# SreenivasVRao/SuperSloMo-VideoInterpolation-PyTorch

Hardware: AMD Instinct MI355X
Metric: interpolated 1280x720 frames/sec (higher is better)
Workload: dtype f32

## Files before the change

include/ssm_hip.h:

```cpp
#ifndef SSM_HIP_H
#define SSM_HIP_H

#include <stddef.h>

#ifdef __cplusplus
extern "C" {
#endif

#define SSM_PADX 4
#define SSM_PADY 3
#define SSM_TAIL_SLACK_FLOATS (1 << 16)

#define SSM_OK 0
#define SSM_E_ARG (-1)
#define SSM_E_LAUNCH (-2)
#define SSM_E_UNSUPPORTED (-3)

#define SSM_FLAG_LRELU 1
#define SSM_FLAG_FP16_FAST 2
#define SSM_FLAG_Q8 4
#define SSM_FLAG_MASK 8

typedef struct ssm_view {
    float *ptr;
// ... 49 lines not shown

int ssm_wino_splitk_plan(int Cin, int Cout, int B, int H, int W, int ups, int BN, int *KS);
int ssm_wino_conv2d_splitk_fwd(ssm_view x1, int C1, ssm_view x2, int C2, const float *w_packed, const float *bias_packed, ssm_view part,
                               int KS, int ups, int B, int H, int W, int Cout, int BN, void *stream);
int ssm_splitk_finish_fwd(ssm_view part, int KS, ssm_view y, ssm_view pool, ssm_view add, int add_div, int B, int C, int H, int W,
                          float slope, int flags, void *stream);
int ssm_conv_splitk_plan(int k, int Cin, int Cout, int B, int H, int W, int *KS);
int ssm_splitk_enable(int wino, int conv);
int ssm_conv2d_splitk_fwd(ssm_view x1, int C1, ssm_view x2, int C2, const float *w_packed, const float *bias_packed, ssm_view part,
                          int KS, int B, int H, int W, int Cout, int k, void *stream);
int ssm_wino_conv2d_add_fwd(ssm_view x1, int C1, ssm_view x2, int C2, const float *w_packed, const float *bias_packed, ssm_view y,
                            ssm_view pool, ssm_view add, int add_div, int B, int H, int W, int Cout, float slope, int flags,
                            void *stream);
int ssm_wino_conv2d_ups_add_fwd(ssm_view a, int C1, ssm_view b, int C2, const float *w_packed, const float *bias_packed, ssm_view y,
                                ssm_view add, int add_div, int B, int H, int W, int Cout, float slope, int flags, void *stream);

int ssm_wino4_plan(int Cin, int Cout, int B, int H, int W, int ups, int *kind, int *BN, int *CK);
int ssm_wino4_preferred(int Cin, int Cout, int B, int H, int W, int ups);
double ssm_wino_estimate(int Cin, int Cout, int B, int H, int W, int ups);
int ssm_wino4_force_kind(int kind);
size_t ssm_wino4_packed_weight_floats(int Cout, int Cin);
int ssm_wino4_pack_weights(const float *w_oihw, const float *bias, float *w_packed, float *bias_packed, int Cout, int Cin, void *stream);
int ssm_wino4_conv2d_add_fwd(ssm_view x1, int C1, ssm_view x2, int C2, const float *w_packed, const float *bias_packed, ssm_view y,
                             ssm_view pool, ssm_view add, int add_div, int B, int H, int W, int Cout, float slope, int flags,
                             void *stream);
int ssm_wino4_conv2d_ups_add_fwd(ssm_view a, int C1, ssm_view b, int C2, const float *w_packed, const float *bias_packed, ssm_view y,
                                 ssm_view add, int add_div, int B, int H, int W, int Cout, float slope, int flags, void *stream);
#define SSM_WINO4_BORDER_TH 16
#define SSM_WINO4_BORDER_TW 32
int ssm_wino4_conv2d_shuffle_fwd(ssm_view x1, int C1, ssm_view x2, int C2, const float *w_packed, const float *bias_packed, ssm_view y, int B,
                                 int H, int W, int Cout4, float slope, int flags, void *stream);
int ssm_wino4_conv2d_ups_border_fwd(ssm_view a, int C1, ssm_view b, int C2, const float *w_packed, const float *bias_packed, ssm_view y, int B,
                                    int H, int W, int Cout, float slope, int flags, void *stream);

int ssm_wino1d_plan(int k, int Cin, int Cout, int B, int H, int W, int *kind, int *BN, int *CK);
int ssm_wino1d_force_kind(int kind);
size_t ssm_wino1d_packed_weight_floats(int Cout, int CinP, int k, int BN);
int ssm_wino1d_pack_weights(const float *w_oihw, const float *bias, float *w_packed, float *bias_packed, int Cout, int Cin,
                            int CinP, int k, int BN, void *stream);
int ssm_wino1d_conv2d_add_fwd(ssm_view x, int Cin, const float *w_packed, const float *bias_packed, ssm_view y, ssm_view pool,
                              ssm_view add, int add_div, int B, int H, int W, int Cout, int k, float slope, int flags, void *stream);

int ssm_wino7_plan(int Cin, int Cout, int B, int H, int W, int *kind);
int ssm_wino7_force_kind(int kind);
size_t ssm_wino7_packed_weight_floats(int Cout, int Cin);
int ssm_wino7_pack_weights(const float *w_oihw, const float *bias, float *w_packed, float *bias_packed, int Cout, int Cin, void *stream);
int ssm_wino7_conv2d_add_fwd(ssm_view x, int Cin, const float *w_packed, const float *bias_packed, ssm_view y, ssm_view pool,
                             ssm_view add, int add_div, int B, int H, int W, int Cout, float slope, int flags, void *stream);

int ssm_wino5_plan(int Cin, int Cout, int B, int H, int W, int *kind);
int ssm_wino5_force_kind(int kind);
size_t ssm_wino5_packed_weight_floats(int Cout, int CinP);
int ssm_wino5_pack_weights(const float *w_oihw, const float *bias, float *w_packed, float *bias_packed, int Cout, int Cin, int CinP,
                           void *stream);
int ssm_wino5_conv2d_add_fwd(ssm_view x, int Cin, const float *w_packed, const float *bias_packed, ssm_view y, ssm_view pool,
                             ssm_view add, int add_div, int B, int H, int W, int Cout, float slope, int flags, void *stream);

enum { SSM_PACK_DIRECT = 0, SSM_PACK_WINO = 1, SSM_PACK_WINO1D = 2, SSM_PACK_WINO4 = 3, SSM_PACK_WINO7 = 4, SSM_PACK_WINO5 = 5 };
typedef struct {
    const float *w;
    const float *bias;
    float *wp, *bp;
    int Cout, Cin, CinP, k, BN, algo, transposed, nbias;
    long long first, total;
} ssm_pack32_job;
int ssm_pack32_weights_batch(const ssm_pack32_job *jobs_device, int n_jobs, long long total_elements, void *stream);
// ... 199 lines not shown
```

superslomo-videointerpolation-pytorch_amd/ssm_amd/engine.py:

```python
import os

import torch

from . import hipbind as hb
from .weights import RECURRENT_HIDDEN, RECURRENT_LAYERS, param_key, recurrent_convs, unet_layers


class KernelTimer:

    def __init__(self):
        self.spans = []

    def span(self, family, name, flops=0.0, nbytes=0.0, issued=None):
        e0, e1 = torch.cuda.Event(enable_timing=True), torch.cuda.Event(enable_timing=True)
        self.spans.append((family, name, flops, nbytes, e0, e1, flops if issued is None else issued))
        return e0, e1

    def summary(self):
        out = {}
        for fam, name, fl, nb, e0, e1, isd in self.spans:
            d = out.setdefault(fam, {"ms": 0.0, "flops": 0.0, "issued": 0.0, "bytes": 0.0, "launches": 0, "by_name": {}})
            ms = e0.elapsed_time(e1)
            d["ms"] += ms
            d["flops"] += fl
# ... 5 lines not shown
            n[1] += fl
            n[2] += 1
        return out


MODES = ("f32", "f32w", "f16x3", "f16", "f16f8")


def base_mode(mode):
    return "f32" if mode == "f32w" else mode


HOIST_PAIR_PARTS = os.environ.get("SSM_HOIST", "1") != "0"

WINO_SKIP = frozenset(n for n in os.environ.get("SSM_WINO_SKIP", "").split(",") if n)

WINO1D = os.environ.get("SSM_WINO1D", "57")


WINO7 = os.environ.get("SSM_WINO7", "1")
WINO5 = os.environ.get("SSM_WINO5", "1")


WINO4 = os.environ.get("SSM_WINO4", "1")


TRAIN_WINO4 = os.environ.get("SSM_TRAIN_WINO4", "1")
TRAIN_FWD_BLOCKED = os.environ.get("SSM_TRAIN_FWD_BLOCKED", "1")


WINO4_SUBPIXEL = tuple(n for n in os.environ.get("SSM_WINO4_SUBPIXEL", "conv11a").split(",") if n not in ("", "0"))


def wino4_enabled(name):
    return WINO4 not in ("0", "") and (WINO4 == "1" or name in WINO4.split(","))


def wino1d_enabled(k):
    return k in (5, 7) and str(k) in WINO1D


def choose_algo(name, ci, co, k, nb, h, w, ups, wino, wino1d, wino4=None, blocked2d=None):
    skip = name in WINO_SKIP or "all" in WINO_SKIP or name == "final_conv"
    wino4 = wino1d if wino4 is None else wino4
    blocked2d = wino1d if blocked2d is None else blocked2d
    if blocked2d and not skip and k == 7 and WINO7 not in ("0", "") and hb.wino7_supported(ci, co, h, w, k):
        return "wino7"
    if blocked2d and not skip and k == 5 and WINO5 not in ("0", "") and ci % 4 == 0 and hb.wino5_supported(ci, co, h, w, k):
        return "wino5"
    if wino1d and not skip and wino1d_enabled(k) and hb.wino1d_supported(ci, co, h, w, k):
        return "wino1d"
    if wino and not skip and hb.wino_supported(ci, co, h, w, k):
        if (wino4 and wino4_enabled(name) and hb.wino4_supported(ci, co, h, w, k)
                and (WINO4 != "1" or hb.wino4_preferred(ci, co, nb, h, w, ups))):
            return "wino4"
        return "wino"
    return "direct"


_ALGO_CLASS = {"direct": lambda: hb.PackedConv, "wino": lambda: hb.PackedWino, "wino4": lambda: hb.PackedWino4, "wino1d": lambda: hb.PackedWino1d,
               "wino7": lambda: hb.PackedWino7, "wino5": lambda: hb.PackedWino5}
ISSUED_FACTOR = {"direct": lambda k: 1.0, "wino": lambda k: 16.0 / 36.0, "wino4": lambda k: 36.0 / 144.0,
                 "wino1d": lambda k: 8.0 / 14.0 if k == 7 else 8.0 / 20.0, "wino7": lambda k: 196.0 / 784.0,
                 "wino5": lambda k: 64.0 / 400.0}


def issued_factor(pk):
    return ISSUED_FACTOR.get(getattr(pk, "algo", "direct"), ISSUED_FACTOR["direct"])(pk.k)


def conv_fn(pk, ups=False):
    if pk.algo == "wino7":
        return hb.conv2d_wino7
    if pk.algo == "wino5":
        return hb.conv2d_wino5
    if pk.algo == "wino1d":
        return hb.conv2d_wino1d
    if pk.algo == "wino4":
        return hb.conv2d_ups_wino4 if ups else hb.conv2d_wino4
    if pk.algo == "wino":
        return hb.conv2d_ups_wino if ups else hb.conv2d_wino
    return hb.conv2d_ups if ups else hb.conv2d


POOLED = ("conv1b", "conv2b", "conv3b", "conv4b", "conv5b")
_SCALE = (("conv10", 2), ("conv11", 1), ("conv1", 1), ("conv2", 2), ("conv3", 4), ("conv4", 8), ("conv5", 16),
          ("conv6", 32), ("conv7", 16), ("conv8", 8), ("conv9", 4), ("fuse_conv", 1), ("final_conv", 1))


def layer_scale(name):
    for prefix, s in _SCALE:
        if name.startswith(prefix):
            return s
    raise KeyError(name)


class UNetPlan:
    timer = None
    RESCALE_EVERY = int(os.environ.get("SSM_RESCALE_EVERY", "256"))
    fast_layers = frozenset()

    DECODER = ("conv7a", "conv7b", "conv8a", "conv8b", "conv9a", "conv9b", "conv10a", "conv10b", "conv11a", "conv11b",
               "fuse_conv", "final_conv")
    ENCODER_T = ("c1", "c2", "c3", "c4", "c5", "c6")
# ... 90 lines not shown
        batchable = self.q8 and all(t.is_cuda and t.dtype == torch.float32 and t.is_contiguous() for t in tensors)
        self._refreshes = getattr(self, "_refreshes", 0) + 1
        if self._refreshes % self.RESCALE_EVERY == 0:
            self.scales, self._pack = {}, None
        if batchable and getattr(self, "_pack", None) is not None and self._pack[0] == hb.PackBatch.key(tensors):
            self._pack[1].run()
            if getattr(self, "rnn", None) is not None:
                self.rnn.refresh_weights(state_dict)
            return
        batch32 = (not self.hl8 and not self.hoist and os.environ.get("SSM_PACK_BATCH", "1") != "0"
                   and all(t.is_cuda and t.dtype == torch.float32 and t.is_contiguous() for t in tensors))
        if batch32 and getattr(self, "_pack32", None) is not None and self._pack32[0] == hb.PackBatch.key(tensors):
            self._pack32[1].run()
            if "final_conv" in self.layers:
                self.final_wb = (state_dict[param_key("final_conv", "weight")].detach(), state_dict[param_key("final_conv", "bias")].detach())
            if getattr(self, "rnn", None) is not None:
                self.rnn.refresh_weights(state_dict)
            return
        for name, (ci, co, k) in self.layers.items():
            w = state_dict[param_key(name, "weight")].to(device=self.device, dtype=torch.float32)
            b = state_dict[param_key(name, "bias")].to(device=self.device, dtype=torch.float32)
            if check_shapes:
                assert tuple(w.shape) == (co, ci, k, k), "%s: weight shape %s != %s" % (name, tuple(w.shape), (co, ci, k, k))
            s = layer_scale(name)
            if name == "final_conv":
                self.final_wb = (w.contiguous(), b.contiguous())
            if self.hl8:
                self.pk[name] = hb.PackedConv16(w, b, self.W // s, q8=self.q8, ups=self.fuse_up and name in self.UPS,
                                                scale=self.scales.get(name))
                self.scales.setdefault(name, self.pk[name].scale)
            else:
                nb = self.Bd if name in self.DECODER else self.B
                ups = self.fuse_up and name in self.UPS
                cls = _ALGO_CLASS[choose_algo(name, ci, co, k, nb, self.H // s, self.W // s, ups, self.wino, self.wino1d, self.wino4, self.blocked2d)]()
                if self.hoist and name == "conv1a":
                    zb = torch.zeros_like(b)
                    self.pk[name] = cls(w[:, 3:13].contiguous(), b, nb, self.H // s, self.W // s)
                    self.pk_pair[name] = cls(torch.cat([w[:, 13:16], w[:, 0:3]], 1).contiguous(), zb, self.hoist[0], self.H // s, self.W // s)
                elif self.hoist and name == "conv7a" and self.cross:
                    zb = torch.zeros_like(b)
                    self.pk[name] = cls(w[:, :512].contiguous(), b, nb, self.H // s, self.W // s, ups=ups)
                    self.pk_pair[name] = cls(w[:, 512:].contiguous(), zb, self.hoist[0], self.H // s, self.W // s, ups=ups)
                elif (ups and cls is hb.PackedWino4 and name in WINO4_SUBPIXEL and not self.twins
                      and hb.subpixel_wino4_supported(ci, co, self.H // s, self.W // s)):
                    self.pk[name] = hb.PackedSubpixelWino4(w, b, nb, self.H // s, self.W // s)
                    batch32 = False
                else:
                    self.pk[name] = cls(w, b, nb, self.H // s, self.W // s, pool=name in POOLED, ups=ups)
        for pkk in list(self.pk.values()) + list(getattr(self, "pk_pair", {}).values()):
            if self.wino and isinstance(pkk, hb.PackedConv):
                pkk.split_ok = True
        self._pack32 = None
        if batch32:
            entries = [(self.pk[name], state_dict[param_key(name, "weight")], state_dict[param_key(name, "bias")], False)
                       for name in self.layers]
            self._pack32 = (hb.PackBatch.key(tensors), hb.PackBatch32(entries, self.device))
        self._pack = None
        if batchable:
            entries = [(self.pk[name], state_dict[param_key(name, "weight")], state_dict[param_key(name, "bias")], False)
                       for name in self.layers]
            self._pack = (hb.PackBatch.key(tensors), hb.PackBatch(entries, self.device))
        if getattr(self, "rnn", None) is not None:
            self.rnn.refresh_weights(state_dict)

    def _v(self, name, **kw):
        if self._b0 and name in self.ENCODER_T:
            kw["b0"] = self._b0
        return self.t[name].view(**kw)

    def _conv(self, name, src, dst, pool=None, src2=None, lrelu=True):
        pk = self.pk[name]
        s = self.t[src]
        d = self.t[dst]
        c2 = self.t[src2].C if src2 else 0
        tm = self.timer
        if tm is not None:
            fl = 2.0 * self._Bcur * s.H * s.W * pk.cout * pk.cin * pk.k * pk.k
            e0, e1 = tm.span("conv", "s%d.%s" % (self.stage, name), fl, issued=fl * issued_factor(pk))
            e0.record()
        v = self._v
        if self.hl8:
            final = name == "final_conv"
            y32 = v(dst) if final else (self.f32[dst].view() if self.twins else None)
            hb.conv2d_hl8(v(src), s.G * 8, v(src2) if src2 else None, c2, pk, None if final else v(dst),
# ... 593 lines not shown
```

superslomo-videointerpolation-pytorch_amd/ssm_amd/hipbind.py:

```python
import ctypes
import os
import threading

import torch

_HERE = os.path.dirname(os.path.abspath(__file__))
LIB_PATH = os.environ.get("SSM_HIP_LIB") or os.path.join(os.path.dirname(_HERE), "lib", "libssm_hip.so")

SSM_PADX = 4
SSM_PADY = 3
SSM_TAIL_SLACK_FLOATS = 1 << 16
SSM_FLAG_LRELU = 1
SSM_FLAG_MASK = 8


class SsmView(ctypes.Structure):
    _fields_ = [("ptr", ctypes.c_void_p), ("sb", ctypes.c_longlong), ("sc", ctypes.c_longlong),
                ("sh", ctypes.c_int)]


NULL_VIEW = SsmView(None, 0, 0, 0)


class SsmHView(ctypes.Structure):
# ... 19 lines not shown
    "ssm_pack_weights": (_c_int, [_vp, _vp, _vp, _vp, _c_int, _c_int, _c_int, _c_int, _c_int, _vp]),
    "ssm_conv2d_fwd": (_c_int, [SsmView, _c_int, SsmView, _c_int, _vp, _vp, SsmView, SsmView, _c_int, _c_int,
                                _c_int, _c_int, _c_int, _c_float, _c_int, _vp]),
    "ssm_conv2d_add_fwd": (_c_int, [SsmView, _c_int, SsmView, _c_int, _vp, _vp, SsmView, SsmView, SsmView, _c_int, _c_int, _c_int,
                                    _c_int, _c_int, _c_int, _c_float, _c_int, _vp]),
    "ssm_conv2d_ups_add_fwd": (_c_int, [SsmView, _c_int, SsmView, _c_int, _vp, _vp, SsmView, SsmView, _c_int, _c_int, _c_int, _c_int,
                                        _c_int, _c_float, _c_int, _vp]),
    "ssm_wino_conv2d_add_fwd": (_c_int, [SsmView, _c_int, SsmView, _c_int, _vp, _vp, SsmView, SsmView, SsmView, _c_int, _c_int, _c_int,
                                         _c_int, _c_int, _c_float, _c_int, _vp]),
    "ssm_wino_conv2d_ups_add_fwd": (_c_int, [SsmView, _c_int, SsmView, _c_int, _vp, _vp, SsmView, SsmView, _c_int, _c_int, _c_int, _c_int,
                                             _c_int, _c_float, _c_int, _vp]),
    "ssm_wino_plan": (_c_int, [_c_int, _c_int, _c_int, _c_int, _c_int, _c_int, _ip, _ip, _ip]),
    "ssm_wino_splitk_plan": (_c_int, [_c_int, _c_int, _c_int, _c_int, _c_int, _c_int, _c_int, _ip]),
    "ssm_conv_splitk_plan": (_c_int, [_c_int, _c_int, _c_int, _c_int, _c_int, _c_int, _ip]),
    "ssm_conv2d_splitk_fwd": (_c_int, [SsmView, _c_int, SsmView, _c_int, _vp, _vp, SsmView, _c_int, _c_int, _c_int, _c_int, _c_int, _c_int, _vp]),
    "ssm_wino_conv2d_splitk_fwd": (_c_int, [SsmView, _c_int, SsmView, _c_int, _vp, _vp, SsmView, _c_int, _c_int, _c_int, _c_int, _c_int, _c_int,
                                            _c_int, _vp]),
    "ssm_splitk_finish_fwd": (_c_int, [SsmView, _c_int, SsmView, SsmView, SsmView, _c_int, _c_int, _c_int, _c_int, _c_int, _c_float, _c_int, _vp]),
    "ssm_wino_force_kind": (_c_int, [_c_int]),
    "ssm_wino_packed_weight_floats": (_sz, [_c_int, _c_int, _c_int]),
    "ssm_wino_pack_weights": (_c_int, [_vp, _vp, _vp, _vp, _c_int, _c_int, _c_int, _vp]),
    "ssm_pack32_weights_batch": (_c_int, [_vp, _c_int, ctypes.c_longlong, _vp]),
    "ssm_pack32_wino_tiles_batch": (_c_int, [_vp, _c_int, ctypes.c_longlong, _c_int, _vp]),
    "ssm_wino4_plan": (_c_int, [_c_int, _c_int, _c_int, _c_int, _c_int, _c_int, _ip, _ip, _ip]),
    "ssm_wino4_force_kind": (_c_int, [_c_int]),
    "ssm_wino4_preferred": (_c_int, [_c_int, _c_int, _c_int, _c_int, _c_int, _c_int]),
    "ssm_wino_estimate": (ctypes.c_double, [_c_int, _c_int, _c_int, _c_int, _c_int, _c_int]),
    "ssm_wino4_packed_weight_floats": (_sz, [_c_int, _c_int]),
    "ssm_wino4_pack_weights": (_c_int, [_vp, _vp, _vp, _vp, _c_int, _c_int, _vp]),
    "ssm_wino4_conv2d_add_fwd": (_c_int, [SsmView, _c_int, SsmView, _c_int, _vp, _vp, SsmView, SsmView, SsmView, _c_int, _c_int, _c_int,
                                          _c_int, _c_int, _c_float, _c_int, _vp]),
    "ssm_wino4_conv2d_ups_add_fwd": (_c_int, [SsmView, _c_int, SsmView, _c_int, _vp, _vp, SsmView, SsmView, _c_int, _c_int, _c_int, _c_int,
                                              _c_int, _c_float, _c_int, _vp]),
    "ssm_wino4_conv2d_shuffle_fwd": (_c_int, [SsmView, _c_int, SsmView, _c_int, _vp, _vp, SsmView, _c_int, _c_int, _c_int, _c_int, _c_float, _c_int, _vp]),
    "ssm_wino4_conv2d_ups_border_fwd": (_c_int, [SsmView, _c_int, SsmView, _c_int, _vp, _vp, SsmView, _c_int, _c_int, _c_int, _c_int, _c_float, _c_int,
                                                 _vp]),
    "ssm_wino1d_plan": (_c_int, [_c_int, _c_int, _c_int, _c_int, _c_int, _c_int, _ip, _ip, _ip]),
    "ssm_wino1d_force_kind": (_c_int, [_c_int]),
    "ssm_wino1d_packed_weight_floats": (_sz, [_c_int, _c_int, _c_int, _c_int]),
    "ssm_wino1d_pack_weights": (_c_int, [_vp, _vp, _vp, _vp, _c_int, _c_int, _c_int, _c_int, _c_int, _vp]),
    "ssm_wino1d_conv2d_add_fwd": (_c_int, [SsmView, _c_int, _vp, _vp, SsmView, SsmView, SsmView, _c_int, _c_int, _c_int, _c_int, _c_int,
                                           _c_int, _c_float, _c_int, _vp]),
    "ssm_wino5_plan": (_c_int, [_c_int, _c_int, _c_int, _c_int, _c_int, _ip]),
    "ssm_wino5_force_kind": (_c_int, [_c_int]),
    "ssm_wino5_packed_weight_floats": (_sz, [_c_int, _c_int]),
    "ssm_wino5_pack_weights": (_c_int, [_vp, _vp, _vp, _vp, _c_int, _c_int, _c_int, _vp]),
    "ssm_wino5_conv2d_add_fwd": (_c_int, [SsmView, _c_int, _vp, _vp, SsmView, SsmView, SsmView, _c_int, _c_int, _c_int, _c_int, _c_int,
                                          _c_float, _c_int, _vp]),
    "ssm_wino7_plan": (_c_int, [_c_int, _c_int, _c_int, _c_int, _c_int, _ip]),
    "ssm_wino7_force_kind": (_c_int, [_c_int]),
    "ssm_wino7_packed_weight_floats": (_sz, [_c_int, _c_int]),
    "ssm_wino7_pack_weights": (_c_int, [_vp, _vp, _vp, _vp, _c_int, _c_int, _vp]),
    "ssm_wino7_conv2d_add_fwd": (_c_int, [SsmView, _c_int, _vp, _vp, SsmView, SsmView, SsmView, _c_int, _c_int, _c_int, _c_int, _c_int,
                                          _c_float, _c_int, _vp]),
    "ssm_wino_conv2d_fwd": (_c_int, [SsmView, _c_int, SsmView, _c_int, _vp, _vp, SsmView, SsmView, _c_int, _c_int, _c_int, _c_int,
                                     _c_float, _c_int, _vp]),
    "ssm_wino_conv2d_ups_fwd": (_c_int, [SsmView, _c_int, SsmView, _c_int, _vp, _vp, SsmView, _c_int, _c_int, _c_int, _c_int,
                                         _c_float, _c_int, _vp]),
    "ssm_conv16_config": (_c_int, [_c_int, _c_int, _c_int, _ip, _ip]),
    "ssm_packed16_weight_halves": (_sz, [_c_int, _c_int, _c_int, _c_int]),
    "ssm_pack16_weights": (_c_int, [_vp, _vp, _vp, _vp, _c_int, _c_int, _c_int, _c_int, _c_int, _c_int, _c_float, _vp]),
    "ssm_conv2d_hl8_fwd": (_c_int, [SsmHView, _c_int, SsmHView, _c_int, _vp, _vp, _c_float, SsmHView, SsmView, SsmHView,
                                    _c_int, _c_int, _c_int, _c_int, _c_int, _c_float, _c_int, _vp]),
    "ssm_conv16q_config": (_c_int, [_c_int, _c_int, _c_int, _ip, _ip]),
    "ssm_conv16q_ups_config": (_c_int, [_c_int, _c_int, _ip, _ip]),
    "ssm_packed16q_weight_bytes": (_sz, [_c_int, _c_int, _c_int, _c_int, _c_int]),
# ... 501 lines not shown
def subpixel_wino4_supported(cin, cout, H, W):
    ty, tx = H // WINO4_BORDER_TH, W // WINO4_BORDER_TW
    return (cin % 4 == 0 and cout % 32 == 0 and H % WINO4_BORDER_TH == 0 and W % WINO4_BORDER_TW == 0 and ty >= 4 and tx >= 4
            and ((ty - 2) * WINO4_BORDER_TH // 2) % 16 == 0 and ((tx - 2) * WINO4_BORDER_TW // 2) % 32 == 0)


class PackedSubpixelWino4:

    algo = "wino4"

    def __init__(self, weight, bias, B, H, W):
        from .subpixel import effective_filter
        self.cout, self.cin, self.k = weight.shape[0], weight.shape[1], 3
        assert subpixel_wino4_supported(self.cin, self.cout, H, W), "sub-pixel F(4x4,3x3): unsupported shape"
        self.border = PackedWino4(weight, bias, B, H, W, ups=True)
        e = effective_filter(weight.detach().to(torch.float32), "int", "int")
        e = e.view(4, self.cout, self.cin, 3, 3).permute(1, 0, 2, 3, 4).reshape(4 * self.cout, self.cin, 3, 3).contiguous()
        self.inner = PackedWino4(e, bias.detach().to(torch.float32).repeat_interleave(4).contiguous(), B, H // 2, W // 2)
        self.w, self.b = self.border.w, self.border.b
        self.ups, self.cin_p, self.bn, self.ck = True, self.cin, self.border.bn, self.border.ck


def conv2d_ups_subpixel_wino4(a_view, c1, b_view, c2, pk, y_view, B, H, W, lrelu=True, slope=0.1):
    lib = load()
    flags = SSM_FLAG_LRELU if lrelu else 0
    y0, x0 = WINO4_BORDER_TH // 2, WINO4_BORDER_TW // 2
    h, w = H // 2 - 2 * y0, W // 2 - 2 * x0
    check(lib.ssm_wino4_conv2d_shuffle_fwd(a_view(y0, x0), c1, b_view(y0, x0) if b_view is not None else NULL_VIEW, c2, pk.inner.w.data_ptr(),
                                           pk.inner.b.data_ptr(), y_view(2 * y0, 2 * x0), B, h, w, 4 * pk.cout, slope, flags, stream_ptr()))
    check(lib.ssm_wino4_conv2d_ups_border_fwd(a_view(0, 0), c1, b_view(0, 0) if b_view is not None else NULL_VIEW, c2, pk.border.w.data_ptr(),
                                              pk.border.b.data_ptr(), y_view(0, 0), B, H, W, pk.cout, slope, flags, stream_ptr()))


def wino1d_plan(k, cin, cout, B, H, W):
    lib = load()
    kind, bn, ck = ctypes.c_int(0), ctypes.c_int(0), ctypes.c_int(0)
    check(lib.ssm_wino1d_plan(k, cin, cout, B, H, W, ctypes.byref(kind), ctypes.byref(bn), ctypes.byref(ck)))
    return kind.value, bn.value, ck.value


def wino1d_supported(cin, cout, H, W, k):
    return k in (5, 7) and cout % 32 == 0


class PackedWino1d:

    algo = "wino1d"

    def __init__(self, weight, bias, B, H, W, pool=False, ups=False):
        require_device(weight, "conv weight")
        require_device(bias, "conv bias")
        assert not ups, "the 7x7 / 5x5 layers have no fused-upsample form"
        self.cout, self.cin, self.k = weight.shape[0], weight.shape[1], weight.shape[2]
        assert self.k in (5, 7) and weight.shape[3] == self.k, "the 1-D Winograd form is for 7x7 and 5x5 filters"
        self.ups = False
        _, self.bn, self.ck = wino1d_plan(self.k, self.cin, self.cout, B, H, W)
        self.cin_p = (self.cin + self.ck - 1) // self.ck * self.ck
        lib = load()
        nw = lib.ssm_wino1d_packed_weight_floats(self.cout, self.cin_p, self.k, self.bn)
        nb = lib.ssm_packed_bias_floats(self.cout, self.bn)
        self.w = torch.empty(nw, dtype=torch.float32, device=weight.device)
        self.b = torch.empty(nb, dtype=torch.float32, device=weight.device)
        wc, bc = weight.detach().contiguous(), bias.detach().contiguous()
        check(lib.ssm_wino1d_pack_weights(wc.data_ptr(), bc.data_ptr(), self.w.data_ptr(), self.b.data_ptr(), self.cout, self.cin,
                                          self.cin_p, self.k, self.bn, stream_ptr()))

# ... 309 lines not shown
```

Baseline: 390.6.

## Add low-resolution GEMM path for fused-upsample 3x3 convolutions

Adds a new path for 3x3 convolutions that follow a bilinear 2x upsample. It runs the convolution as an MFMA GEMM over the nine taps at low resolution into a scratch buffer, then a combine kernel applies the fixed bilinear weights, bias, residual add and leaky ReLU at full resolution. This cuts the multiply work compared with convolving the upsampled tensor. In exchange it writes and reads a 9×Cout scratch intermediate and adds a second launch. It is enabled by default only for the large-channel layer shapes that the heuristic prefers.

```diff
diff --git a/include/ssm_hip.h b/include/ssm_hip.h
--- a/include/ssm_hip.h
+++ b/include/ssm_hip.h
@@ -105,6 +105,15 @@
                                  int H, int W, int Cout4, float slope, int flags, void *stream);
 int ssm_wino4_conv2d_ups_border_fwd(ssm_view a, int C1, ssm_view b, int C2, const float *w_packed, const float *bias_packed, ssm_view y, int B,
                                     int H, int W, int Cout, float slope, int flags, void *stream);
+
+int ssm_upgemm_supported(int Cin, int Cout, int H, int W, int k);
+int ssm_upgemm_preferred(int Cin, int Cout, int B, int h, int w);
+int ssm_upgemm_force_kind(int kind);
+size_t ssm_upgemm_packed_weight_floats(int Cout, int Cin);
+int ssm_upgemm_pack_weights(const float *w_oihw, float *w_packed, int Cout, int Cin, void *stream);
+size_t ssm_upgemm_scratch_floats(int Cout, int B, int h, int w);
+int ssm_upgemm_conv2d_ups_add_fwd(ssm_view a, int C1, ssm_view b, int C2, const float *w_packed, const float *bias, ssm_view scratch, ssm_view y,
+                                  ssm_view add, int add_div, int B, int H, int W, int Cout, float slope, int flags, void *stream);
 
 int ssm_wino1d_plan(int k, int Cin, int Cout, int B, int H, int W, int *kind, int *BN, int *CK);
 int ssm_wino1d_force_kind(int kind);
diff --git a/superslomo-videointerpolation-pytorch_amd/csrc/ssm_upgemm.hip b/superslomo-videointerpolation-pytorch_amd/csrc/ssm_upgemm.hip
--- /dev/null
+++ b/superslomo-videointerpolation-pytorch_amd/csrc/ssm_upgemm.hip
@@ -0,0 +1,491 @@
+#include "ssm_common.h"
+#include "ssm_device.h"
+
+#include <atomic>
+#include <cstdlib>
+
+namespace {
+
+constexpr int BM = 128;
+constexpr int CK = 16;
+
+struct GemmParams {
+    const float *src1;
+    const float *src2;
+    long long sb1, sb2;
+    long long sc;
+    int sh;
+    int C1, Cin, CinP;
+    const float *wpk;
+    float *dst;
+    long long dsb, dsc;
+    int dsh;
+    int h, w, M;
+    int tilesX, tilesY, NB;
+};
+
+template <int MTY_, int MTX_>
+struct GCfg {
+    static constexpr int MTY = MTY_, MTX = MTX_, MT = MTY_ * MTX_, NT = 2, WN = 2, WY = 2;
+    static constexpr int GW = 8, GH = 4;
+    static constexpr int TH = MTY * GH * WY, TW = MTX * GW;
+    static constexpr int TW4 = TW / 4;
+    static constexpr int WSZ = CK * BM, PSZ = CK * TH * TW;
+    static constexpr int NWQ = WSZ / 4, NDQ = PSZ / 4, NQ = NWQ + NDQ;
+    static constexpr int NG = NQ / 64, NI = NG / 4;
+    static constexpr int STAGE = WSZ + PSZ;
+    static constexpr int BYTES = 2 * STAGE * 4;
+    static_assert(TW == 16, "the patch swizzle below is written for 16-float rows");
+    static_assert(NWQ % 64 == 0 && NQ % 256 == 0, "every wave-instruction is all filter or all patch; equal shares per wave");
+    static_assert(BYTES <= 65536, "LDS budget (two workgroups per CU)");
+};
+
+__device__ __forceinline__ int swz_piece(int r, int j) { return j ^ (((r >> 1) & 1) << 1); }
+
+template <class C, bool RAGGED>
+__global__ __launch_bounds__(256, 2) void upgemm_kernel(const GemmParams p) {
+    extern __shared__ __attribute__((aligned(16))) float lds[];
+    constexpr int NT = C::NT, MT = C::MT, GW = C::GW, GH = C::GH, TH = C::TH, TW = C::TW;
+
+    const int tid = threadIdx.x;
+    const int lane = tid & 63, l31 = lane & 31, half = lane >> 5;
+    const int gy = l31 / GW, gx = l31 % GW;
+    const int wid = __builtin_amdgcn_readfirstlane(tid >> 6);
+    const int wn = wid % C::WN, wy = wid / C::WN;
+
+    int id = ssm_xcd_tile(blockIdx.x, gridDim.x);
+    const int nb = id % p.NB;
+    id /= p.NB;
+    const int tx = id % p.tilesX;
+    id /= p.tilesX;
+    const int ty = id % p.tilesY;
+    const int b = id / p.tilesY;
+    const int x0 = tx * TW, y0 = ty * TH;
+    const int nchunks = p.CinP / CK;
+
+    const long long porg = (long long)y0 * p.sh + x0;
+    const float *pbase1 = p.src1 + (long long)b * p.sb1 + porg;
+    const float *pbase2 = p.src2 + (long long)b * p.sb2 + porg;
+    const float *wbase = p.wpk + (long long)nb * p.CinP * BM;
+
+    int off[C::NI];
+    int pch[C::NI];
+#pragma unroll
+    for (int i = 0; i < C::NI; ++i) {
+        const int q = (i * 4 + wid) * 64 + lane;
+        if (q < C::NWQ) {
+            off[i] = q * 4;
+            pch[i] = 0;
+        } else {
+            const int qq = q - C::NWQ;
+            const int c = qq / (TH * C::TW4);
+            const int rem = qq - c * (TH * C::TW4);
+            const int r = rem / C::TW4, j = swz_piece(r, rem % C::TW4);
+            pch[i] = c;
+            off[i] = (RAGGED ? 0 : (int)(c * p.sc)) + r * p.sh + 4 * j;
+        }
+    }
+    const unsigned lds0 = (unsigned)(size_t)(__attribute__((address_space(3))) void *)lds;
+    auto issue_k = [&](int ch, int stage, int k) {
+        const int c0 = ch * CK;
+        const float *wb = wbase + (long long)c0 * BM;
+        const unsigned lsb = lds0 + (unsigned)(stage * C::STAGE) * 4u;
+#pragma unroll
+        for (int wv = 0; wv < 4; ++wv) {
+            const int g = 4 * k + wv;
+            if (wv == wid) {
+                const bool is_w = g * 64 < C::NWQ;
+                if (is_w) {
+                    lds_dma16(wb, off[k] * 4, lsb + (unsigned)g * 1024u);
+                } else if constexpr (!RAGGED) {
+                    const float *pb = (c0 < p.C1) ? pbase1 + (long long)c0 * p.sc : pbase2 + (long long)(c0 - p.C1) * p.sc;
+                    lds_dma16(pb, off[k] * 4, lsb + (unsigned)g * 1024u);
+                } else {
+                    const int cg = c0 + pch[k];
+                    const float *pb = cg < p.C1 ? pbase1 + (long long)cg * p.sc : (cg < p.Cin ? pbase2 + (long long)(cg - p.C1) * p.sc : pbase1);
+                    SSM_GLDS16(pb + off[k], lds + stage * C::STAGE + g * 256);
+                }
+            }
+        }
+    };
+
+    f32x16 acc[NT][MT];
+#pragma unroll
+    for (int n = 0; n < NT; ++n)
+#pragma unroll
+        for (int m = 0; m < MT; ++m)
+#pragma unroll
+            for (int r = 0; r < 16; ++r) acc[n][m][r] = 0.f;
+
+    const int aBase = half * BM + wn * (NT * 32) + l31;
+    const int sw = ((gy >> 1) & 1) * 8;
+    int bBase[C::MTX];
+#pragma unroll
+    for (int mx = 0; mx < C::MTX; ++mx) bBase[mx] = C::WSZ + half * (TH * TW) + (wy * C::MTY * GH + gy) * TW + ((mx * GW) ^ sw) + gx;
+
+#pragma unroll
+    for (int k = 0; k < C::NI; ++k) issue_k(0, 0, k);
+    for (int ch = 0; ch < nchunks; ++ch) {
+        wait_vmcnt<0>();
+        __syncthreads();
+        const bool dma_next = ch + 1 < nchunks;
+        const float *stg = lds + (ch & 1) * C::STAGE;
+        constexpr int S = CK / 2;
+        float a[2][NT], bv[2][MT];
+        auto fetch = [&](int s, int buf) {
+#pragma unroll
+            for (int n = 0; n < NT; ++n) a[buf][n] = stg[aBase + 2 * s * BM + n * 32];
+#pragma unroll
+            for (int my = 0; my < C::MTY; ++my)
+#pragma unroll
+                for (int mx = 0; mx < C::MTX; ++mx) bv[buf][my * C::MTX + mx] = stg[bBase[mx] + (2 * s * TH + my * GH) * TW];
+        };
+        fetch(0, 0);
+#pragma unroll
+        for (int s = 0; s < S; ++s) {
+#pragma unroll
+            for (int n = 0; n < NT; ++n)
+#pragma unroll
+                for (int m = 0; m < MT; ++m) {
+                    acc[n][m] = __builtin_amdgcn_mfma_f32_32x32x2f32(a[s & 1][n], bv[s & 1][m], acc[n][m], 0, 0, 0);
+                    if (n == 0 && m == 0) {
+                        __builtin_amdgcn_sched_barrier(0);
+                        if (s + 1 < S) fetch(s + 1, (s + 1) & 1);
+                        if (s < C::NI && dma_next) issue_k(ch + 1, (ch + 1) & 1, s);
+                        __builtin_amdgcn_sched_barrier(0);
+                    }
+                }
+            __builtin_amdgcn_sched_barrier(0);
+        }
+        static_assert(C::NI <= S, "one DMA instruction per k-step");
+    }
+
+    const int xbase = x0 + gx, ybase = y0 + wy * (C::MTY * GH) + gy;
+    float *dstb = p.dst + (long long)b * p.dsb;
+    const int m0 = nb * BM + wn * (NT * 32);
+    const unsigned pbase = 4u * ((unsigned)(4 * half) * (unsigned)p.dsc + (unsigned)ybase * (unsigned)p.dsh + (unsigned)xbase);
+    bool pok[MT];
+#pragma unroll
+    for (int m = 0; m < MT; ++m) pok[m] = ybase + (m / C::MTX) * GH < p.h && xbase + (m % C::MTX) * GW < p.w;
+#pragma unroll
+    for (int n = 0; n < NT; ++n) {
+        if (m0 + n * 32 < p.M) {
+#pragma unroll
+            for (int r = 0; r < 16; ++r) {
+                const int mu = m0 + n * 32 + (r & 3) + 8 * (r >> 2);
+                float *bp = dstb + (long long)mu * p.dsc;
+#pragma unroll
+                for (int m = 0; m < MT; ++m) {
+                    float *bpm = bp + ((m / C::MTX) * GH) * p.dsh + (m % C::MTX) * GW;
+                    if (pok[m]) store_sbase(bpm, pbase, acc[n][m][r]);
+                }
+            }
+        }
+    }
+}
+
+using G16 = GCfg<2, 2>;
+using G8 = GCfg<1, 2>;
+enum GemmKind { KG16, KG8, NGKIND };
+constexpr int kTH[NGKIND] = {G16::TH, G8::TH}, kTW[NGKIND] = {G16::TW, G8::TW};
+
+std::atomic<int> g_force_kind{-1};
+
+int pick_kind(int h, int w) {
+    const int forced = g_force_kind.load();
+    if (forced >= 0 && forced < NGKIND) return forced;
+    long long best = 0;
+    int kd = 0;
+    for (int i = 0; i < NGKIND; ++i) {
+        const long long px = (long long)((h + kTH[i] - 1) / kTH[i]) * kTH[i] * ((w + kTW[i] - 1) / kTW[i]) * kTW[i];
+        if (i == 0 || px < best) {
+            best = px;
+            kd = i;
+        }
+    }
+    return kd;
+}
+
+template <class C>
+int launch_gemm(GemmParams &p, int B, bool ragged, hipStream_t st) {
+    p.tilesX = (p.w + C::TW - 1) / C::TW;
+    p.tilesY = (p.h + C::TH - 1) / C::TH;
+    const long long blocks = (long long)p.tilesX * p.tilesY * p.NB * B;
+    if (blocks <= 0 || blocks > 0x7fffffffLL) {
+        ssm::set_error("upgemm: grid of %lld workgroups out of range", blocks);
+        return SSM_E_ARG;
+    }
+    if (ragged) SSM_LAUNCH((upgemm_kernel<C, true>), dim3((unsigned)blocks), dim3(256), C::BYTES, st, p);
+    else SSM_LAUNCH((upgemm_kernel<C, false>), dim3((unsigned)blocks), dim3(256), C::BYTES, st, p);
+    return ssm::check_launch("ssm_upgemm_conv2d_ups_add_fwd (gemm)");
+}
+
+struct CombineParams {
+    const float *y;
+    long long ysb, ysc;
+    int ysh;
+    const float *bias;
+    float *dst;
+    long long dsb, dsc;
+    int dsh;
+    const float *add;
+    long long asb, asc;
+    int ash, adiv;
+    int h, w, Cout, nq;
+    long long total;
+    float slope;
+};
+
+template <bool W4>
+__global__ __launch_bounds__(256) void upgemm_combine_kernel(const CombineParams p) {
+    const long long t = (long long)blockIdx.x * 256 + threadIdx.x;
+    if (t >= p.total) return;
+    long long r = t;
+    const int q = (int)(r % p.nq);
+    r /= p.nq;
+    const int i = (int)(r % p.h);
+    r /= p.h;
+    const int co = (int)(r % p.Cout);
+    const int b = (int)(r / p.Cout);
+    const int j0 = 4 * q;
+    const int W = 2 * p.w;
+
+    const int rowm = max(i - 1, 0), rowp = min(i + 1, p.h - 1);
+    const int cm = max(j0 - 1, 0), cp = min(j0 + 4, p.w - 1);
+    const float mt = i > 0 ? 1.f : 0.f, mb = i < p.h - 1 ? 1.f : 0.f;
+    const float *yb = p.y + (long long)b * p.ysb + (long long)co * p.ysc;
+    const long long tapc = (long long)p.Cout * p.ysc;
+
+    float acc[2][8];
+#pragma unroll
+    for (int d = 0; d < 2; ++d)
+#pragma unroll
+        for (int x = 0; x < 8; ++x) acc[d][x] = 0.f;
+
+    auto load_row = [&](const float *plane, int row, float (&c)[6]) {
+        const float *rp = plane + (long long)row * p.ysh;
+        c[0] = rp[cm];
+        if constexpr (W4) {
+            const f32x4 v = *(const f32x4 *)(rp + j0);
+            c[1] = v[0], c[2] = v[1], c[3] = v[2], c[4] = v[3];
+        } else {
+#pragma unroll
+            for (int k = 0; k < 4; ++k) c[1 + k] = rp[min(j0 + k, p.w - 1)];
+        }
+        c[5] = rp[cp];
+    };
+#pragma unroll
+    for (int v = 0; v < 3; ++v) {
+        float V[2][6];
+        float c[6];
+        const float *pl = yb + (long long)v * tapc;
+        load_row(pl, rowm, c);
+#pragma unroll
+        for (int k = 0; k < 6; ++k) V[0][k] = (0.75f * mt) * c[k], V[1][k] = 0.25f * c[k];
+        load_row(pl, i, c);
+#pragma unroll
+        for (int k = 0; k < 6; ++k) V[0][k] += (0.25f * mt) * c[k], V[1][k] += 0.75f * c[k];
+        pl = yb + (long long)(3 + v) * tapc;
+        load_row(pl, rowm, c);
+#pragma unroll
+        for (int k = 0; k < 6; ++k) V[0][k] += 0.25f * c[k];
+        load_row(pl, i, c);
+#pragma unroll
+        for (int k = 0; k < 6; ++k) V[0][k] += 0.75f * c[k], V[1][k] += 0.75f * c[k];
+        load_row(pl, rowp, c);
+#pragma unroll
+        for (int k = 0; k < 6; ++k) V[1][k] += 0.25f * c[k];
+        pl = yb + (long long)(6 + v) * tapc;
+        load_row(pl, i, c);
+#pragma unroll
+        for (int k = 0; k < 6; ++k) V[0][k] += 0.75f * c[k], V[1][k] += (0.25f * mb) * c[k];
+        load_row(pl, rowp, c);
+#pragma unroll
+        for (int k = 0; k < 6; ++k) V[0][k] += 0.25f * c[k], V[1][k] += (0.75f * mb) * c[k];
+#pragma unroll
+        for (int x = 0; x < 8; ++x) {
+            const int tt = x + v - 1;
+            const int k = (tt + 2) / 2 - 1;
+            const bool odd = (tt & 1) != 0;
+            const int ia = odd ? k + 1 : k, ib = ia + 1;
+            const float wa = odd ? 0.75f : 0.25f, wb = odd ? 0.25f : 0.75f;
+            const int Q = 2 * j0 + tt;
+            const bool in = Q >= 0 && Q < W;
+#pragma unroll
+            for (int d = 0; d < 2; ++d) {
+                const float u = wa * V[d][ia] + wb * V[d][ib];
+                acc[d][x] += in ? u : 0.f;
+            }
+        }
+    }
+    const float bs = p.bias[co];
+    const float sl = p.slope;
+    float *dp = p.dst + (long long)b * p.dsb + (long long)co * p.dsc + (long long)(2 * i) * p.dsh + 2 * j0;
+    const float *ap = p.add ? p.add + (long long)(b / p.adiv) * p.asb + (long long)co * p.asc + (long long)(2 * i) * p.ash + 2 * j0 : nullptr;
+    const int nx = min(8, W - 2 * j0);
+#pragma unroll
+    for (int d = 0; d < 2; ++d) {
+        float o[8];
+#pragma unroll
+        for (int x = 0; x < 8; ++x) o[x] = acc[d][x] + bs;
+        if (ap) {
+            const float *a = ap + (long long)d * p.ash;
+            if (W4 || nx == 8) {
+                const f32x4 a0 = *(const f32x4 *)a, a1 = *(const f32x4 *)(a + 4);
+#pragma unroll
+                for (int x = 0; x < 4; ++x) o[x] += a0[x], o[4 + x] += a1[x];
+            } else {
+#pragma unroll
+                for (int x = 0; x < 8; ++x)
+                    if (x < nx) o[x] += a[x];
+            }
+        }
+#pragma unroll
+        for (int x = 0; x < 8; ++x) o[x] = fmaxf(o[x], o[x] * sl);
+        float *dr = dp + (long long)d * p.dsh;
+        if (W4 || nx == 8) {
+            f32x4 s0, s1;
+#pragma unroll
+            for (int x = 0; x < 4; ++x) s0[x] = o[x], s1[x] = o[4 + x];
+            *(f32x4 *)dr = s0;
+            *(f32x4 *)(dr + 4) = s1;
+        } else {
+#pragma unroll
+            for (int x = 0; x < 8; ++x)
+                if (x < nx) dr[x] = o[x];
+        }
+    }
+}
+
+__global__ void upgemm_pack_kernel(const float *__restrict__ w, float *__restrict__ wp, int Cout, int Cin, int CinP, long long total) {
+    const long long i = (long long)blockIdx.x * blockDim.x + threadIdx.x;
+    if (i >= total) return;
+    const int n = (int)(i % BM);
+    const long long r = i / BM;
+    const int ci = (int)(r % CinP);
+    const int m = (int)(r / CinP) * BM + n;
+    float v = 0.f;
+    if (m < 9 * Cout && ci < Cin) {
+        const int tap = m / Cout, co = m - tap * Cout;
+        v = w[((long long)co * Cin + ci) * 9 + tap];
+    }
+    wp[i] = v;
+}
+
+inline int round_up(int a, int b) { return (a + b - 1) / b * b; }
+
+}
+
+extern "C" int ssm_upgemm_supported(int Cin, int Cout, int H, int W, int k) {
+    return k == 3 && Cin > 0 && Cout > 0 && Cout % 32 == 0 && H > 0 && W > 0 && H % 2 == 0 && W % 2 == 0;
+}
+
+extern "C" int ssm_upgemm_preferred(int Cin, int Cout, int B, int h, int w) {
+    if (!ssm_upgemm_supported(Cin, Cout, 2 * h, 2 * w, 3) || B <= 0) return 0;
+    const long long px = (long long)B * h * w;
+    if (Cin >= 512 && Cout >= 512) return px <= 4096;
+    if (Cin >= 1024 && Cout >= 256) return px >= 32768;
+    if (Cin >= 512 && Cout >= 128) return px >= 131072;
+    return 0;
+}
+
+extern "C" int ssm_upgemm_force_kind(int kind) {
+    g_force_kind.store(kind >= 0 && kind < NGKIND ? kind : -1);
+    return NGKIND;
+}
+
+extern "C" size_t ssm_upgemm_packed_weight_floats(int Cout, int Cin) {
+    return (size_t)round_up(9 * Cout, BM) * (size_t)round_up(Cin, CK);
+}
+
+extern "C" int ssm_upgemm_pack_weights(const float *w_oihw, float *w_packed, int Cout, int Cin, void *stream) {
+    SSM_REQUIRE(w_oihw && w_packed, "upgemm pack_weights: null pointer");
+    SSM_REQUIRE(Cout > 0 && Cin > 0 && Cout % 32 == 0, "upgemm pack_weights: bad sizes (Cout = %d must be a multiple of 32)", Cout);
+    const long long total = (long long)ssm_upgemm_packed_weight_floats(Cout, Cin);
+    SSM_LAUNCH(upgemm_pack_kernel, dim3((unsigned)((total + 255) / 256)), dim3(256), 0, (hipStream_t)stream, w_oihw, w_packed, Cout, Cin,
+               round_up(Cin, CK), total);
+    return ssm::check_launch("ssm_upgemm_pack_weights");
+}
+
+extern "C" size_t ssm_upgemm_scratch_floats(int Cout, int B, int h, int w) {
+    return (size_t)B * 9 * (size_t)Cout * (size_t)h * (size_t)round_up(w, 4);
+}
+
+extern "C" int ssm_upgemm_conv2d_ups_add_fwd(ssm_view a, int C1, ssm_view b, int C2, const float *w_packed, const float *bias, ssm_view scratch,
+                                             ssm_view y, ssm_view add, int add_div, int B, int H, int W, int Cout, float slope, int flags,
+                                             void *stream) {
+    SSM_REQUIRE(B > 0 && C1 > 0 && C2 >= 0, "upgemm: bad batch / channel counts");
+    SSM_REQUIRE(ssm_upgemm_supported(C1 + C2, Cout, H, W, 3), "upgemm: unsupported problem (Cout = %d must be a multiple of 32, H x W = %d x %d even)",
+                Cout, H, W);
+    SSM_REQUIRE(a.ptr && y.ptr && scratch.ptr && w_packed && bias, "upgemm: null pointer");
+    const int h = H / 2, w = W / 2;
+    SSM_REQUIRE(ssm::aligned16(a.ptr) && a.sh % 4 == 0 && a.sc % 4 == 0 && a.sb % 4 == 0, "upgemm: input 1 is not a padded-plane view (16-byte alignment)");
+    SSM_REQUIRE(a.sh >= w + 2 * SSM_PADX, "upgemm: input 1 row stride %d leaves no frame for w=%d", a.sh, w);
+    SSM_REQUIRE(ssm::aligned16(w_packed), "upgemm: packed filter must be 16-byte aligned");
+    if (C2 > 0) {
+        SSM_REQUIRE(b.ptr && ssm::aligned16(b.ptr) && b.sb % 4 == 0, "upgemm: input 2 is not a padded-plane view");
+        SSM_REQUIRE(b.sh == a.sh && b.sc == a.sc, "upgemm: cat sources must share row/channel strides");
+    }
+    SSM_REQUIRE(4LL * ((long long)CK * a.sc + 32LL * a.sh) < 0x7fffffffLL, "upgemm: channel stride too large");
+    SSM_REQUIRE(ssm::aligned16(scratch.ptr) && scratch.sh % 4 == 0 && scratch.sh >= w && scratch.sc % 4 == 0 && scratch.sb % 4 == 0 &&
+                    scratch.sc >= (long long)h * scratch.sh && scratch.sb >= 9LL * Cout * scratch.sc,
+                "upgemm: scratch view too small or misaligned for 9 x %d planes of %d x %d", Cout, h, w);
+    SSM_REQUIRE(4LL * (4 * scratch.sc + (long long)(h + 32) * scratch.sh) < 0x7fffffffLL, "upgemm: scratch plane too large for 32-bit offsets");
+    SSM_REQUIRE(ssm::aligned16(y.ptr) && y.sh % 4 == 0 && y.sc % 4 == 0 && y.sb % 4 == 0, "upgemm: output is not a padded-plane view (16-byte alignment)");
+    if (add.ptr) {
+        SSM_REQUIRE(add_div >= 1 && B % add_div == 0, "upgemm: the addend serves %d batch entries each, batch %d is no multiple", add_div, B);
+        SSM_REQUIRE(ssm::aligned16(add.ptr) && add.sh % 4 == 0 && add.sc % 4 == 0 && add.sb % 4 == 0, "upgemm: addend is not a padded-plane view");
+    }
+    hipStream_t st = (hipStream_t)stream;
+
+    GemmParams g;
+    g.src1 = a.ptr;
+    g.src2 = C2 > 0 ? b.ptr : a.ptr;
+    g.sb1 = a.sb;
+    g.sb2 = C2 > 0 ? b.sb : 0;
+    g.sc = a.sc;
+    g.sh = a.sh;
+    g.C1 = C1;
+    g.Cin = C1 + C2;
+    g.CinP = round_up(C1 + C2, CK);
+    g.wpk = w_packed;
+    g.dst = scratch.ptr;
+    g.dsb = scratch.sb;
+    g.dsc = scratch.sc;
+    g.dsh = scratch.sh;
+    g.h = h;
+    g.w = w;
+    g.M = 9 * Cout;
+    g.NB = (g.M + BM - 1) / BM;
+    const bool ragged = C1 % CK != 0 || (C1 + C2) % CK != 0;
+    const int kd = pick_kind(h, w);
+    const int rc = kd == KG16 ? launch_gemm<G16>(g, B, ragged, st) : launch_gemm<G8>(g, B, ragged, st);
+    if (rc != SSM_OK) return rc;
+
+    CombineParams c;
+    c.y = scratch.ptr;
+    c.ysb = scratch.sb;
+    c.ysc = scratch.sc;
+    c.ysh = scratch.sh;
+    c.bias = bias;
+    c.dst = y.ptr;
+    c.dsb = y.sb;
+    c.dsc = y.sc;
+    c.dsh = y.sh;
+    c.add = add.ptr;
+    c.asb = add.ptr ? add.sb : 0;
+    c.asc = add.ptr ? add.sc : 0;
+    c.ash = add.ptr ? add.sh : 0;
+    c.adiv = add.ptr ? add_div : 1;
+    c.h = h;
+    c.w = w;
+    c.Cout = Cout;
+    c.nq = (w + 3) / 4;
+    c.total = (long long)B * Cout * h * c.nq;
+    c.slope = (flags & SSM_FLAG_LRELU) ? slope : 1.f;
+    const long long blocks = (c.total + 255) / 256;
+    SSM_REQUIRE(blocks > 0 && blocks <= 0x7fffffffLL, "upgemm: combine grid of %lld workgroups out of range", blocks);
+    if (w % 4 == 0) SSM_LAUNCH(upgemm_combine_kernel<true>, dim3((unsigned)blocks), dim3(256), 0, st, c);
+    else SSM_LAUNCH(upgemm_combine_kernel<false>, dim3((unsigned)blocks), dim3(256), 0, st, c);
+    return ssm::check_launch("ssm_upgemm_conv2d_ups_add_fwd (combine)");
+}
diff --git a/superslomo-videointerpolation-pytorch_amd/ssm_amd/engine.py b/superslomo-videointerpolation-pytorch_amd/ssm_amd/engine.py
--- a/superslomo-videointerpolation-pytorch_amd/ssm_amd/engine.py
+++ b/superslomo-videointerpolation-pytorch_amd/ssm_amd/engine.py
@@ -61,6 +61,13 @@
 WINO4_SUBPIXEL = tuple(n for n in os.environ.get("SSM_WINO4_SUBPIXEL", "conv11a").split(",") if n not in ("", "0"))
 
 
+UPGEMM = os.environ.get("SSM_UPGEMM", "1")
+
+
+def upgemm_enabled(name):
+    return UPGEMM not in ("0", "") and (UPGEMM == "1" or name in UPGEMM.split(","))
+
+
 def wino4_enabled(name):
     return WINO4 not in ("0", "") and (WINO4 == "1" or name in WINO4.split(","))
 
@@ -69,10 +76,13 @@
     return k in (5, 7) and str(k) in WINO1D
 
 
-def choose_algo(name, ci, co, k, nb, h, w, ups, wino, wino1d, wino4=None, blocked2d=None):
+def choose_algo(name, ci, co, k, nb, h, w, ups, wino, wino1d, wino4=None, blocked2d=None, upgemm=True):
     skip = name in WINO_SKIP or "all" in WINO_SKIP or name == "final_conv"
     wino4 = wino1d if wino4 is None else wino4
     blocked2d = wino1d if blocked2d is None else blocked2d
+    if (upgemm and wino and wino1d and ups and not skip and k == 3 and upgemm_enabled(name) and hb.upgemm_supported(ci, co, h, w, k)
+            and (UPGEMM != "1" or hb.upgemm_preferred(ci, co, nb, h, w))):
+        return "upgemm"
     if blocked2d and not skip and k == 7 and WINO7 not in ("0", "") and hb.wino7_supported(ci, co, h, w, k):
         return "wino7"
     if blocked2d and not skip and k == 5 and WINO5 not in ("0", "") and ci % 4 == 0 and hb.wino5_supported(ci, co, h, w, k):
@@ -88,10 +98,10 @@
 
 
 _ALGO_CLASS = {"direct": lambda: hb.PackedConv, "wino": lambda: hb.PackedWino, "wino4": lambda: hb.PackedWino4, "wino1d": lambda: hb.PackedWino1d,
-               "wino7": lambda: hb.PackedWino7, "wino5": lambda: hb.PackedWino5}
+               "wino7": lambda: hb.PackedWino7, "wino5": lambda: hb.PackedWino5, "upgemm": lambda: hb.PackedUpGemm}
 ISSUED_FACTOR = {"direct": lambda k: 1.0, "wino": lambda k: 16.0 / 36.0, "wino4": lambda k: 36.0 / 144.0,
                  "wino1d": lambda k: 8.0 / 14.0 if k == 7 else 8.0 / 20.0, "wino7": lambda k: 196.0 / 784.0,
-                 "wino5": lambda k: 64.0 / 400.0}
+                 "wino5": lambda k: 64.0 / 400.0, "upgemm": lambda k: 9.0 / 36.0}
 
 
 def issued_factor(pk):
@@ -99,6 +109,9 @@
 
 
 def conv_fn(pk, ups=False):
+    if pk.algo == "upgemm":
+        assert ups, "the low-res GEMM form is for the fused-upsample layers"
+        return hb.conv2d_ups_upgemm
     if pk.algo == "wino7":
         return hb.conv2d_wino7
     if pk.algo == "wino5":
@@ -255,7 +268,12 @@
             else:
                 nb = self.Bd if name in self.DECODER else self.B
                 ups = self.fuse_up and name in self.UPS
-                cls = _ALGO_CLASS[choose_algo(name, ci, co, k, nb, self.H // s, self.W // s, ups, self.wino, self.wino1d, self.wino4, self.blocked2d)]()
+                algo_args = (name, ci, co, k, nb, self.H // s, self.W // s, ups, self.wino, self.wino1d, self.wino4, self.blocked2d)
+                cls = _ALGO_CLASS[choose_algo(*algo_args)]()
+                pair_cls = cls
+                if cls is hb.PackedUpGemm:
+                    pair_cls = _ALGO_CLASS[choose_algo(*algo_args, upgemm=False)]()
+                    batch32 = False
                 if self.hoist and name == "conv1a":
                     zb = torch.zeros_like(b)
                     self.pk[name] = cls(w[:, 3:13].contiguous(), b, nb, self.H // s, self.W // s)
@@ -263,7 +281,7 @@
                 elif self.hoist and name == "conv7a" and self.cross:
                     zb = torch.zeros_like(b)
                     self.pk[name] = cls(w[:, :512].contiguous(), b, nb, self.H // s, self.W // s, ups=ups)
-                    self.pk_pair[name] = cls(w[:, 512:].contiguous(), zb, self.hoist[0], self.H // s, self.W // s, ups=ups)
+                    self.pk_pair[name] = pair_cls(w[:, 512:].contiguous(), zb, self.hoist[0], self.H // s, self.W // s, ups=ups)
                 elif (ups and cls is hb.PackedWino4 and name in WINO4_SUBPIXEL and not self.twins
                       and hb.subpixel_wino4_supported(ci, co, self.H // s, self.W // s)):
                     self.pk[name] = hb.PackedSubpixelWino4(w, b, nb, self.H // s, self.W // s)
@@ -273,6 +291,13 @@
         for pkk in list(self.pk.values()) + list(getattr(self, "pk_pair", {}).values()):
             if self.wino and isinstance(pkk, hb.PackedConv):
                 pkk.split_ok = True
+        ug = [(pkk, name) for name, pkk in self.pk.items() if isinstance(pkk, hb.PackedUpGemm)]
+        if ug:
+            need = max(pkk.scratch_floats(self.Bd, self.H // layer_scale(name), self.W // layer_scale(name)) for pkk, name in ug)
+            if getattr(self, "_upgemm_scratch", None) is None or self._upgemm_scratch.numel() < need:
+                self._upgemm_scratch = torch.empty(need, dtype=torch.float32, device=self.device)
+            for pkk, _ in ug:
+                pkk.scratch = self._upgemm_scratch
         self._pack32 = None
         if batch32:
             entries = [(self.pk[name], state_dict[param_key(name, "weight")], state_dict[param_key(name, "bias")], False)
diff --git a/superslomo-videointerpolation-pytorch_amd/ssm_amd/hipbind.py b/superslomo-videointerpolation-pytorch_amd/ssm_amd/hipbind.py
--- a/superslomo-videointerpolation-pytorch_amd/ssm_amd/hipbind.py
+++ b/superslomo-videointerpolation-pytorch_amd/ssm_amd/hipbind.py
@@ -75,6 +75,14 @@
                                           _c_int, _c_int, _c_float, _c_int, _vp]),
     "ssm_wino4_conv2d_ups_add_fwd": (_c_int, [SsmView, _c_int, SsmView, _c_int, _vp, _vp, SsmView, SsmView, _c_int, _c_int, _c_int, _c_int,
                                               _c_int, _c_float, _c_int, _vp]),
+    "ssm_upgemm_supported": (_c_int, [_c_int, _c_int, _c_int, _c_int, _c_int]),
+    "ssm_upgemm_preferred": (_c_int, [_c_int, _c_int, _c_int, _c_int, _c_int]),
+    "ssm_upgemm_force_kind": (_c_int, [_c_int]),
+    "ssm_upgemm_packed_weight_floats": (_sz, [_c_int, _c_int]),
+    "ssm_upgemm_pack_weights": (_c_int, [_vp, _vp, _c_int, _c_int, _vp]),
+    "ssm_upgemm_scratch_floats": (_sz, [_c_int, _c_int, _c_int, _c_int]),
+    "ssm_upgemm_conv2d_ups_add_fwd": (_c_int, [SsmView, _c_int, SsmView, _c_int, _vp, _vp, SsmView, SsmView, SsmView, _c_int, _c_int, _c_int,
+                                               _c_int, _c_int, _c_float, _c_int, _vp]),
     "ssm_wino4_conv2d_shuffle_fwd": (_c_int, [SsmView, _c_int, SsmView, _c_int, _vp, _vp, SsmView, _c_int, _c_int, _c_int, _c_int, _c_float, _c_int, _vp]),
     "ssm_wino4_conv2d_ups_border_fwd": (_c_int, [SsmView, _c_int, SsmView, _c_int, _vp, _vp, SsmView, _c_int, _c_int, _c_int, _c_int, _c_float, _c_int,
                                                  _vp]),
@@ -642,6 +650,53 @@
                                               pk.border.b.data_ptr(), y_view(0, 0), B, H, W, pk.cout, slope, flags, stream_ptr()))
 
 
+def upgemm_supported(cin, cout, H, W, k=3):
+    return bool(load().ssm_upgemm_supported(cin, cout, H, W, k))
+
+
+def upgemm_preferred(cin, cout, B, H, W):
+    return bool(load().ssm_upgemm_preferred(cin, cout, B, H // 2, W // 2))
+
+
+def upgemm_scratch_view(buf, cout, h, w):
+    wr = (w + 3) // 4 * 4
+    return SsmView(buf.data_ptr(), 9 * cout * h * wr, h * wr, wr)
+
+
+class PackedUpGemm:
+
+    algo = "upgemm"
+
+    def __init__(self, weight, bias, B, H, W, pool=False, ups=True):
+        require_device(weight, "conv weight")
+        require_device(bias, "conv bias")
+        assert ups and not pool, "the low-res GEMM form is for the fused-upsample layers"
+        self.cout, self.cin, self.k = weight.shape[0], weight.shape[1], weight.shape[2]
+        if not upgemm_supported(self.cin, self.cout, H, W, self.k):
+            raise RuntimeError("low-res GEMM form: unsupported layer (%d -> %d, k = %d, output %d x %d)" % (self.cin, self.cout, self.k, H, W))
+        self.ups, self.cin_p, self.bn, self.ck = True, self.cin, 128, 16
+        lib = load()
+        self.w = torch.empty(lib.ssm_upgemm_packed_weight_floats(self.cout, self.cin), dtype=torch.float32, device=weight.device)
+        self.b = bias.detach().contiguous().clone()
+        check(lib.ssm_upgemm_pack_weights(weight.detach().contiguous().data_ptr(), self.w.data_ptr(), self.cout, self.cin, stream_ptr()))
+        self.scratch = None
+
+    def scratch_floats(self, B, H, W):
+        return load().ssm_upgemm_scratch_floats(self.cout, B, H // 2, W // 2)
+
+
+def conv2d_ups_upgemm(a, c1, b, c2, pk, y, B, H, W, lrelu=True, slope=0.1, add=None, add_div=1):
+    lib = load()
+    assert pk.cin == c1 + c2, "packed filter expects %d input channels, got %d" % (pk.cin, c1 + c2)
+    need = pk.scratch_floats(B, H, W)
+    if pk.scratch is None or pk.scratch.numel() < need:
+        pk.scratch = torch.empty(need, dtype=torch.float32, device=pk.w.device)
+    check(lib.ssm_upgemm_conv2d_ups_add_fwd(a, c1, b if b is not None else NULL_VIEW, c2, pk.w.data_ptr(), pk.b.data_ptr(),
+                                            upgemm_scratch_view(pk.scratch, pk.cout, H // 2, W // 2), y,
+                                            add if add is not None else NULL_VIEW, add_div, B, H, W, pk.cout, slope,
+                                            SSM_FLAG_LRELU if lrelu else 0, stream_ptr()))
+
+
 def wino1d_plan(k, cin, cout, B, H, W):
     lib = load()
     kind, bn, ck = ctypes.c_int(0), ctypes.c_int(0), ctypes.c_int(0)
```

New measurement: 398.5 (median of 6 runs). 2.0% higher.
